# dpmerrell/PathMatFac.jl

Hardware: AMD Instinct MI355X
Metric: fit_iters_per_sec (higher is better)
Workload: dtype f32; 1 GPU; fit! epoch on synthetic 200000x50000 matrix (D stored as f32), K=64, Gaussian loss, group-reg X (32 groups) + featureset-ARD Y, adam; rows sharded over 1 GPU(s); full_model=False, M=200000, N=50000, K=64, rows_per_gpu=200000, optimizer=adam, parallelism=single GPU, rccl_ranks=0, collectives_issued=0, column_chunks=1

## Files before the change

include/pmf_hip.h:

```cpp
#ifndef PMF_HIP_H
#define PMF_HIP_H

#include <stdint.h>

#ifdef __cplusplus
extern "C" {
#endif

typedef struct pmf_ctx pmf_ctx;

#define PMF_NOISE_NORMAL 0
#define PMF_NOISE_BERNOULLI 1
#define PMF_NOISE_POISSON 2
#define PMF_NOISE_SQ_HINGE 3

#define PMF_OPT_ADAGRAD 0
#define PMF_OPT_ADAM 1

#define PMF_STORE_F32 0
#define PMF_STORE_BF16 1

#define PMF_TERM_MAX_EPOCHS 0
#define PMF_TERM_LOSS_INCREASE 1
#define PMF_TERM_ABS_TOL 2
// ... 134 lines not shown
int pmf_fit_lbfgs(pmf_ctx *ctx, const pmf_lbfgs_opts *opts, pmf_lbfgs_result *result);
int pmf_debug_lbfgs_direction(pmf_ctx *ctx, int n_pairs, const float *sX, const float *sY, const float *yX,
                              const float *yY, const float *gX, const float *gY, float *pX, float *pY);

int pmf_epoch_begin(pmf_ctx *ctx, const pmf_fit_opts *opts);
int pmf_epoch_step_local(pmf_ctx *ctx, const pmf_fit_opts *opts);
int pmf_epoch_step_shared(pmf_ctx *ctx, const pmf_fit_opts *opts);
int pmf_epoch_loss(pmf_ctx *ctx, double *local_loss, double *shared_terms);

#define PMF_COMM_ID_BYTES 128
#define PMF_COMM_NONE 0
#define PMF_COMM_RCCL 1
#define PMF_COMM_HOST 2
typedef int (*pmf_host_allreduce_fn)(void *user, void *host_buf, int64_t count, int dtype);
int pmf_comm_get_unique_id(void *id_out);
int pmf_comm_init(pmf_ctx *ctx, int rank, int nranks, const void *unique_id);
int pmf_comm_init_host(pmf_ctx *ctx, int rank, int nranks, pmf_host_allreduce_fn fn, void *user);
int pmf_comm_destroy(pmf_ctx *ctx);
int pmf_comm_set_chunks(pmf_ctx *ctx, int n_chunks);
int pmf_comm_allreduce(pmf_ctx *ctx, void *host_buf, int64_t count, int dtype, int op);
int pmf_comm_info(pmf_ctx *ctx, int *rank, int *nranks, int *transport, int *n_chunks, int *reserved_cus,
                  int64_t *n_collectives);

int pmf_debug_last_path(pmf_ctx *ctx, int *bmode, int *layer_path, int *slots, int *xreg, int64_t *plain_tiles);
int pmf_debug_plain_table(pmf_ctx *ctx, int32_t *out, int64_t cap, int64_t *n_rp, int64_t *n_ct);
int pmf_debug_last_kernel(pmf_ctx *ctx, int *kernel);

#define PMF_PASS_EXTENTS_MAX 16
int pmf_debug_pass_extents(pmf_ctx *ctx, int update_X, int update_Y, const int64_t *cap_override, int n_max,
                           const char **names, int64_t *need, int64_t *capacity, int *n);

int pmf_debug_live_bytes(int64_t *device_bytes, int64_t *pinned_bytes);

int pmf_grad_device_ptr(pmf_ctx *ctx, int which, void **ptr, int64_t *n_elements);
int pmf_get_grad(pmf_ctx *ctx, int which, int view, float *out);

int pmf_forward(pmf_ctx *ctx, float *Z_host);

#define PMF_IMPUTE_BATCH 1
#define PMF_IMPUTE_LINK 2
#define PMF_IMPUTE_KEEP_OBSERVED 4
int pmf_impute(pmf_ctx *ctx, int flags, int64_t row_start1, int64_t row_stop1, float *out_host, int64_t ld);
int pmf_impute_device(pmf_ctx *ctx, int flags, int64_t row_start1, int64_t row_stop1, float *out_device, int64_t ld);
int pmf_impute_entries(pmf_ctx *ctx, int flags, int64_t n, const int64_t *rows1, const int64_t *cols1, float *out_host);
int pmf_debug_impute_offset(int64_t row, int64_t col, int64_t ld, int64_t *offset);

typedef struct pmf_sim_opts {
// ... 73 lines not shown
```

pathmatfac.jl_amd/_lib.py:

```python
import ctypes as C
import os
from pathlib import Path

import numpy as np

_HERE = Path(__file__).resolve().parent
LIB_PATH = _HERE / "libpmf_hip.so"

NOISE = {"normal": 0, "bernoulli": 1, "poisson": 2, "bernoulli_sq_hinge": 3, "ordinal_sq_hinge3": 3}
HINGE_THRESHOLDS = {"bernoulli_sq_hinge": (0.0, np.inf, np.inf), "ordinal_sq_hinge3": (-np.inf, -0.5, 0.5)}
OPT = {"adagrad": 0, "adam": 1}
STORE = {"f32": 0, "bf16": 1}
TERM = {0: "max_epochs", 1: "loss_increase", 2: "abs_tol", 3: "rel_tol", 4: "nonfinite"}
IMPUTE_BATCH, IMPUTE_LINK, IMPUTE_KEEP_OBSERVED = 1, 2, 4
DEBATCH_LINK, DEBATCH_FILL_MISSING = 1, 2
PARAM = {"X": 0, "Y": 1, "logsigma": 2, "mu": 3, "logdelta": 4, "theta": 5}


class PMFError(RuntimeError):
    pass


class FitOpts(C.Structure):
    _fields_ = [("update_X", C.c_int32), ("update_Y", C.c_int32), ("update_col_layers", C.c_int32),
# ... 57 lines not shown
    L, Nv = S.shape
    flat = np.flatnonzero(S.ravel())
    rowptr = np.zeros(L + 1, np.int64)
    if Nv:
        np.cumsum(np.bincount(flat // Nv, minlength=L), out=rowptr[1:])
        col = (flat % Nv).astype(np.int32)
    else:
        col = np.zeros(0, np.int32)
    return rowptr, col, S.ravel()[flat].astype(np.float32)


EXPORTS = [
    "pmf_last_error", "pmf_version", "pmf_device_count", "pmf_create", "pmf_destroy", "pmf_set_stream", "pmf_synchronize",
    "pmf_set_data", "pmf_set_data_device", "pmf_set_factors", "pmf_set_X", "pmf_set_Y", "pmf_get_factors",
    "pmf_set_col_params", "pmf_get_col_params", "pmf_set_n_batch_views", "pmf_set_batch_view",
    "pmf_get_batch_view", "pmf_set_noise", "pmf_clear_xreg", "pmf_add_xreg_l2", "pmf_add_xreg_group",
    "pmf_clear_yreg", "pmf_add_yreg_l2", "pmf_add_yreg_group", "pmf_add_yreg_ard", "pmf_add_yreg_fsard",
    "pmf_set_layer_regs", "pmf_set_optimizer", "pmf_set_lr", "pmf_get_lr", "pmf_reset_optimizer_state",
    "pmf_fit", "pmf_epoch_begin", "pmf_epoch_step_local", "pmf_epoch_step_shared", "pmf_epoch_loss",
    "pmf_grad_device_ptr", "pmf_get_grad", "pmf_forward", "pmf_stats", "pmf_kernel_time", "pmf_synth_data",
    "pmf_set_precision", "pmf_get_precision",
    "pmf_comm_get_unique_id", "pmf_comm_init", "pmf_comm_init_host", "pmf_comm_destroy", "pmf_comm_set_chunks",
    "pmf_comm_info", "pmf_comm_allreduce", "pmf_get_opt_state", "pmf_fsard_update_A", "pmf_debug_last_path", "pmf_debug_last_kernel",
    "pmf_debug_pass_extents", "pmf_debug_live_bytes", "pmf_debug_plain_table",
    "pmf_add_xreg_network", "pmf_add_yreg_network", "pmf_get_reg_network_state", "pmf_add_xreg_l1", "pmf_add_yreg_l1",
    "pmf_impute", "pmf_impute_device", "pmf_impute_entries", "pmf_debug_impute_offset",
    "pmf_loss", "pmf_fit_lbfgs", "pmf_debug_lbfgs_direction",
    "pmf_stage_init_logsigma", "pmf_stage_reweight_col_losses", "pmf_get_noise_weights", "pmf_stage_minimal_group_weights",
    "pmf_stage_theta_delta_em",
    "pmf_gram", "pmf_stage_lambda_max", "pmf_stage_whiten", "pmf_stage_rotate_by_svd", "pmf_stage_reorder_by_importance",
    "pmf_debug_postprocess_times",
    "pmf_fsard_update_A_csr",
    "pmf_set_noise_thresholds", "pmf_get_noise_thresholds",
    "pmf_remove_batch_effect", "pmf_remove_batch_effect_device", "pmf_remove_batch_effect_entries",
    "pmf_simulate_data", "pmf_simulate_data_device", "pmf_simulate_data_resident",
]

COMM_ID_BYTES = 128
HOST_ALLREDUCE_FN = C.CFUNCTYPE(C.c_int, C.c_void_p, C.c_void_p, C.c_int64, C.c_int)


def comm_unique_id(lib_path=None):
    lib = load_library(lib_path)
    buf = C.create_string_buffer(COMM_ID_BYTES)
    if lib.pmf_comm_get_unique_id(buf) != 0:
        raise PMFError(lib.pmf_last_error().decode())
    return buf.raw
# ... 683 lines not shown

    def comm_destroy(self):
        self._chk(self.lib.pmf_comm_destroy(self._h))
        self._host_cb = None

    def comm_set_chunks(self, n):
        self._chk(self.lib.pmf_comm_set_chunks(self._h, int(n)))

    def comm_allreduce(self, arr, op="sum"):
        if arr.dtype not in (np.float32, np.float64) or not arr.flags.c_contiguous:
            raise PMFError("comm_allreduce needs a contiguous float32 / float64 array")
        self._chk(self.lib.pmf_comm_allreduce(self._h, arr.ctypes.data_as(C.c_void_p), C.c_int64(arr.size),
                                              1 if arr.dtype == np.float64 else 0, {"sum": 0, "max": 1}[op]))
        return arr

    def comm_info(self):
        r, n, t, ch, cu = C.c_int(0), C.c_int(0), C.c_int(0), C.c_int(0), C.c_int(0)
        nc = C.c_int64(0)
        self._chk(self.lib.pmf_comm_info(self._h, C.byref(r), C.byref(n), C.byref(t), C.byref(ch), C.byref(cu), C.byref(nc)))
        return dict(rank=r.value, nranks=n.value, transport=("none", "rccl", "host")[t.value], n_chunks=ch.value,
                    reserved_cus=cu.value, n_collectives=nc.value)

    def last_path(self):
        b, l, s, x = C.c_int(0), C.c_int(0), C.c_int(0), C.c_int(0)
        pt = C.c_int64(0)
        self._chk(self.lib.pmf_debug_last_path(self._h, C.byref(b), C.byref(l), C.byref(s), C.byref(x), C.byref(pt)))
        return dict(bmode=b.value, layer_path=l.value, slots=s.value, xreg=x.value, plain_tiles=pt.value)

    def plain_table(self):
        n_rp, n_ct = C.c_int64(0), C.c_int64(0)
        self._chk(self.lib.pmf_debug_plain_table(self._h, None, C.c_int64(0), C.byref(n_rp), C.byref(n_ct)))
        out = np.zeros((n_rp.value, n_ct.value + 1), np.int32)
        self._chk(self.lib.pmf_debug_plain_table(self._h, out.ctypes.data_as(C.c_void_p), C.c_int64(out.size), None, None))
        return out

    def last_kernel(self):
        k = C.c_int(0)
        self._chk(self.lib.pmf_debug_last_kernel(self._h, C.byref(k)))
        return k.value

    def pass_extents(self, update_X=False, update_Y=False, capacity_override=None):
        n_max = 16
        names, n = (C.c_char_p * n_max)(), C.c_int(0)
        need, cap = (C.c_int64 * n_max)(), (C.c_int64 * n_max)()
        ov = None
        if capacity_override is not None:
            plain = self.pass_extents(update_X, update_Y)
            unknown = set(capacity_override) - set(plain)
            if unknown:
                raise PMFError(f"pass_extents: unknown buffers {sorted(unknown)}")
# ... 23 lines not shown
```

pathmatfac.jl_amd/csrc/pmf_common.h:

```cpp
#ifndef PMF_COMMON_H
#define PMF_COMMON_H
#include <hip/hip_runtime.h>

#include <cstdint>
#include <type_traits>
#include <unordered_map>

#include "../../include/pmf_hip.h"

int pmf_fail(const char *fmt, ...);
#define HIPCHK(x)                                                                                    \
  do {                                                                                               \
    hipError_t e_ = (x);                                                                             \
    if (e_ != hipSuccess) return pmf_fail("%s failed: %s (%s:%d)", #x, hipGetErrorString(e_), __FILE__, __LINE__); \
  } while (0)
#define PMFCHK(x)          \
  do {                     \
    int r_ = (x);          \
    if (r_ < 0) return r_; \
  } while (0)

typedef std::unordered_map<const void *, size_t> PmfDynLds;
int pmf_ensure_dyn_lds(PmfDynLds *cache, const void *kern, size_t lds);

// ... 39 lines not shown
  const float2 *btab;
  const float2 *btd;
  const uint8_t *pm, *row_slot, *colview;
  int32_t nbs_shift;
  int32_t n_bv;
  double *loss_partial;
  int64_t M, N;
  int32_t n_cseg;
  int32_t want_gx, want_gy;
  unsigned long long *stamps;
  int32_t dbg;
  const ViewDesc *views;
  const char *Xsb, *Ysb;
  int32_t ct0;
  float *gx_part;
  const int32_t *piece_base;
  int64_t gx_slot_stride;
  const float *sb_scale_x, *sb_scale_y;
  const float *htab;
  const int32_t *ptab;
  int32_t ptab_stride;
  int32_t plain;
  int32_t *plain_count;
};

__device__ __forceinline__ int pmf_rowmap(int r, int h) { return (r & 3) + 8 * (r >> 2) + 4 * h; }
__device__ __forceinline__ bool pmf_finite(float y) { return fabsf(y) <= 3.402823466e38f; }

__host__ __device__ __forceinline__ int pmf_meta_kind(int meta) { return meta & 3; }
__host__ __device__ __forceinline__ int pmf_meta_view(int meta) { return (meta >> 2) - 1; }
__host__ __device__ __forceinline__ int64_t pmf_view_index(const ViewDesc &vd, int64_t j, int b) { return (j - vd.c0) * vd.nb + b; }
__host__ __device__ __forceinline__ int64_t pmf_btab_index(const ViewDesc &vd, int64_t j, int b) { return vd.tab_off + pmf_view_index(vd, j, b); }
__device__ __forceinline__ int pmf_row_batch(const int32_t *bor, int64_t M, int v, int64_t i) { return v >= 0 ? bor[(int64_t)v * M + i] : -1; }
__device__ __forceinline__ float2 pmf_batch_dt(const ViewDesc &vd, const float2 *btab, int64_t j, int b) {
  return b >= 0 ? btab[pmf_btab_index(vd, j, b)] : make_float2(1.f, 0.f);
}

#define PMF_HT 8
__device__ __forceinline__ void pmf_hinge_terms(float z, float y, const float *T, float &a, float &b) {
  const int c = (int)fminf(fmaxf(y + 0.5f, 0.f), 3.f);
  const float lo = T[c], hi = T[4 + c];
  a = fmaxf(0.f, 1.f - (z - lo));
  b = fmaxf(0.f, 1.f - (hi - z));
}
__device__ __forceinline__ float pmf_hinge_class(float z, const float4 t) { return (float)((t.x < z) + (t.y < z) + (t.z < z)); }

// ... 386 lines not shown
```

pathmatfac.jl_amd/csrc/pmf_ctx.h:

```cpp
#ifndef PMF_CTX_H
#define PMF_CTX_H
#include <hip/hip_runtime.h>

#include <algorithm>
#include <atomic>
#include <chrono>
#include <cmath>
#include <cstdarg>
#include <cstdio>
#include <cstdlib>
#include <cstring>
#include <memory>
#include <string>
#include <unordered_map>
#include <vector>

#include "pmf_common.h"

int memset_now(void *p, int v, size_t bytes);
inline std::atomic<int64_t> pmf_live_bytes[2];
template <typename T, bool PINNED = false>
struct DevBuf {
  T *p = nullptr;
  size_t n = 0;
// ... 123 lines not shown
  int64_t ptab_bm = 0, ptab_n_rp = 0, ptab_n_ct = 0;
  DevBuf<int32_t> plain_count;
  int64_t last_plain_n = -1;
  int store = PMF_STORE_F32;
  ParamBuf P[6];
  int n_bv = 0;
  std::vector<ViewDesc> views;
  std::vector<int64_t> val_off;
  std::vector<int64_t> bvb_off;
  DevBuf<int32_t> bor;
  DevBuf<float2> btab;
  bool views_dirty = true;
  DevBuf<ViewDesc> d_views;
  DevBuf<float2> LG;
  DevBuf<float> lgrad_part;
  DevBuf<float2> btd;
  bool btd_ok = false;
  int nbs = 16;
  DevBuf<uint8_t> colview;
  std::vector<std::vector<int32_t>> h_bor;
  PanelSlots pslots[3];
  int64_t views_serial = 0;
  int last_kernel = 0;
  int last_bmode = 0, last_layer_path = 0, last_xreg = 0;
  DevBuf<int32_t> d_val_view;
  DevBuf<int32_t> colmeta;
  DevBuf<float> colw;
  DevBuf<float4> colp;
  DevBuf<float4> thr;
  DevBuf<float> htab;
  std::vector<float> h_thr;
  bool mixed = false;
  bool prepared = false;
  DevBuf<float> ard_alpha, ard_beta;
  float ard_scale = 0.f;
  bool has_ard = false;
  bool ard_is_fsard = false;
  int opt_kind = PMF_OPT_ADAGRAD;
  float lr = 1.f, eps = 1e-8f, b1 = 0.9f, b2 = 0.999f;
  bool state_init = false;
  DevBuf<double> loss_partial;
  std::vector<uint8_t> h_kind;
  std::vector<int64_t> noise_s1, noise_e1;
  std::vector<WorkSplit> splits;
  int n_chunks_req = 0;
  DevBuf<float> gx_part;
  DevBuf<int32_t> gx_off, gx_idx;
// ... 152 lines not shown
```

pathmatfac.jl_amd/csrc/pmf_fused.hip.inc:

```

template <int KB, int NW, int RBW = 1>
struct FusedCfg {
  static constexpr int Kp = 32 * KB;
  static constexpr int KpS = Kp + 4;
  static constexpr int SLAB = 32 * Kp;
  static constexpr int YT = PMF_BN * KpS;
  static constexpr int XP = 32 * KpS;
  static constexpr int TT = (RBW - 1) * 1024;
  static constexpr int FIXED = NW * SLAB + NW * RBW * XP + NW * TT + 8 * PMF_BN + 4;
  static constexpr int LDS_BUDGET = 160 * 1024;
  static constexpr int NYB = (2 * YT + FIXED) * 4 + 8 * NW <= LDS_BUDGET ? 2 : 1;
  static constexpr size_t lds_bytes = (sizeof(float) * (NYB * YT + FIXED) + sizeof(double) * NW + 15) / 16 * 16;
  static constexpr size_t lds_batch_extra = PMF_BN * 16 * sizeof(float2) + PMF_PM_BYTES + NW * RBW * 16 * 32;
};

#ifndef PMF_NW4_WAVES
#define PMF_NW4_WAVES 1
#endif
#ifndef PMF_Y1BASE
#define PMF_Y1BASE 1
#endif
template <bool B> struct PmfFlag { static constexpr bool value = B; };
template <int KB, int NW, int RBW, int BMODE, bool MIXED, int GM, bool DB, bool XW = false, bool XR = false>
__global__ __launch_bounds__(64 * NW, (NW == 8 ? 2 : PMF_NW4_WAVES)) void pmf_fused_kernel(const FusedArgs a) {
// ... 94 lines not shown
    }
  }
  constexpr bool Y1BASE = PLAINB && PMF_Y1BASE != 0;
  unsigned g2_lane = (unsigned)(uintptr_t)(lds_cptr)(Ys + 4 * h * KpS + l31);
  if (Y1BASE) asm volatile("" : "+v"(g2_lane));
  auto ho_at = [](const void *base, unsigned &off) {
    if (PLAINB) asm volatile("" : "+v"(off));
    return reinterpret_cast<const char *>(base) + off;
  };
#ifdef PMF_STAMPS
  unsigned long long st_acc[16] = {0, 0, 0, 0, 0, 0, 0, 0, 0, 0, 0, 0, 0, 0, 0, 0};
  unsigned long long st_prev = __builtin_amdgcn_s_memtime();
  const unsigned long long st_t0 = st_prev, st_r0 = __builtin_amdgcn_s_memrealtime();
#endif
  const int wg = pmf_xcd_wg(blockIdx.x, gridDim.x);
  const int64_t w_begin = a.wg_begin[wg];
  const int64_t w_end = a.wg_begin[wg + 1];
  float *myslab = a.gy_slabs + (int64_t)wg * a.slab_stride;
  const int64_t seg_block = a.n_rp * a.tps;
  double lossacc = 0.0;
  int n_plain = 0;
  int seg_cur = -1, pidx = 0, t0_first = 0;
  int gx_slot = (GM == 2) ? 0 : a.piece_base[wg];
  for (int64_t widx = w_begin; widx < w_end;) {
    int cs = (int)(widx / seg_block);
    if (cs > a.n_cseg - 1) cs = a.n_cseg - 1;
    const int tps_cs = cs == a.n_cseg - 1 ? a.n_ct - (a.n_cseg - 1) * a.tps : a.tps;
    const int64_t rem = widx - (int64_t)cs * seg_block;
    const int64_t rp = rem / tps_cs;
    const int ti0 = (int)(rem - rp * tps_cs);
    const int ntiles = (int)(tps_cs - ti0 < w_end - widx ? tps_cs - ti0 : w_end - widx);
    widx += ntiles;
    if (cs != seg_cur) { seg_cur = cs; pidx = 0; t0_first = ti0; } else { ++pidx; }
    bool slab_first = true;
    int pl_b = ntiles, pl_e = ntiles;
    int32_t pl_c0 = 0, pl_c1 = 0;
    if (PLAINB && a.plain) {
      const int64_t c_abs = (int64_t)a.ct0 + (int64_t)cs * a.tps + ti0;
      const bool rag = (c_abs + ntiles) * PMF_BN > N;
      pl_b = pidx == 0 ? ntiles : (pidx == 1 ? (t0_first - ti0 < 0 ? 0 : (t0_first - ti0 < ntiles ? t0_first - ti0 : ntiles)) : 0);
      pl_e = rag ? ntiles - 2 : ntiles;
      if (pl_b < pl_e) {
        const int32_t *pt = a.ptab + rp * a.ptab_stride;
        pl_c0 = pt[c_abs + pl_b];
        pl_c1 = pt[c_abs + (rag ? ntiles - 1 : ntiles)];
      } else {
        pl_b = pl_e = ntiles;
      }
    }
    const int64_t col_begin = ((int64_t)a.ct0 + (int64_t)cs * a.tps + ti0) * BN;
    int64_t row0[RBW], irow_c[RBW];
    bool row_ok[RBW];
#pragma unroll
    for (int rb = 0; rb < RBW; ++rb) {
      row0[rb] = rp * BM + (int64_t)(w * RBW + rb) * 32;
      const int64_t irow = row0[rb] + l31;
      row_ok[rb] = irow < M;
      irow_c[rb] = row_ok[rb] ? irow : (M - 1);
    }

    constexpr int XV = (32 * Kp / 4) / 64;
    float4 xv0[RBW][XV];
#pragma unroll
    for (int rb = 0; rb < RBW; ++rb) {
#pragma unroll
      for (int q = 0; q < XV; ++q) {
        const int e4 = lane + 64 * q;
        const int il = (e4 * 4) / Kp;
        const int64_t ir = row0[rb] + il < M ? row0[rb] + il : M - 1;
        xv0[rb][q] = *reinterpret_cast<const float4 *>(a.X + ir * Kp + (e4 * 4) % Kp);
      }
    }
    f32x16 gx[RBW][KB];
#pragma unroll
    for (int rb = 0; rb < RBW; ++rb)
#pragma unroll
      for (int kb = 0; kb < KB; ++kb)
#pragma unroll
        for (int r = 0; r < 16; ++r) gx[rb][kb][r] = 0.f;
    float4 xf[XR ? KS / 4 : 1];
    float xg[XR ? 8 * NW : 1];

    auto stage_load_y = [&](int64_t jt, int q, float4 (&yv)[YV], float (&sgv)[YV], bool plain = false) {
      const float *yb = a.Y + jt * Kp;
      const float4 *cb = a.colp + jt;
      const int64_t rem = N - jt;
      if (HOIST && !(PLAINB && !plain && rem < BN)) {
        const bool rag = HOZ == 2 && rem < BN;
        yv[q] = *reinterpret_cast<const float4 *>(ho_at(yb, rag ? ho_y[HOZ - 1][q] : ho_y[0][q]));
        sgv[q] = *reinterpret_cast<const float *>(ho_at(cb, rag ? ho_s[HOZ - 1][q] : ho_s[0][q]));
        return;
      }
      const int ncol = rem > BN ? BN : (int)rem;
      int e4 = tid + NT * q;
// ... 150 lines not shown
        const int64_t rem = N - jt_red;
        const int nel = (rem > BN ? BN : (int)rem) * Kp;
        float *sb = myslab + jt_red * Kp;
#pragma unroll
        for (int q = 0; q < RV4; ++q) {
          float4 v = racc[q];
          const float sgj = Csg[(cbuf ^ 1) * BN + eo[q] / Kp];
          v.x *= sgj; v.y *= sgj; v.z *= sgj; v.w *= sgj;
          if (!slab_first) { v.x += gold[q].x; v.y += gold[q].y; v.z += gold[q].z; v.w += gold[q].w; }
          if (in[q] && eo[q] < nel) pmf_store_stream(reinterpret_cast<float4 *>(sb + eo[q]), v);
        }
      }
    };

    bool rows_in[RBW];
    int rb_u[RBW];
    uint32_t tflag[RBW];
#pragma unroll
    for (int rb = 0; rb < RBW; ++rb) {
      const int rb_raw = __builtin_amdgcn_readfirstlane((int)(row0[rb] >> 5));
      rows_in[rb] = rb_raw < a.nRB;
      rb_u[rb] = rows_in[rb] ? rb_raw : (int)a.nRB - 1;
      tflag[rb] = a.tflags[(col_begin >> 5) * a.nRB + rb_u[rb]];
#pragma unroll
      for (int q = 0; q < DCH; ++q) dcur[rb].load(a.D, (col_begin >> 5) * a.nRB + rb_u[rb], lane, q);
    }
    {
      float4 yv[YV], cv;
      float sgv[YV];
      stage_load(col_begin, yv, sgv, cv);
#pragma unroll
      for (int rb = 0; rb < RBW; ++rb)
#pragma unroll
        for (int q = 0; q < XV; ++q) {
          const int e4 = lane + 64 * q;
          const int il = (e4 * 4) / Kp, kf = (e4 * 4) % Kp;
          *reinterpret_cast<float4 *>(Xw[rb] + il * KpS + kf) = row0[rb] + il < M ? xv0[rb][q] : make_float4(0.f, 0.f, 0.f, 0.f);
        }
      stage_store(0, 0, col_begin, yv, sgv, cv);
      if (bt_lds) {
#pragma unroll
        for (int q = 0; q < NBT; ++q) {
          const int e = bt_e(q);
          bt_store(e, pmf_bt_entry(a, a.pm + rp * a.n_bv * 16, col_begin, e, pmf_bt_view(a, col_begin, e)), bt_mu(col_begin, e));
        }
        if (tid < a.n_bv * 16) Pm[tid] = a.pm[rp * a.n_bv * 16 + tid];
        if (h == 0)
#pragma unroll
          for (int rb = 0; rb < RBW; ++rb)
            for (int v = 0; v < a.n_bv; ++v) Bw0[rb * 512 + v * 32 + l31] = a.row_slot[(int64_t)v * M + irow_c[rb]];
      }
    }
    __syncthreads();
    if (XR) {
      const float4 *xr0 = reinterpret_cast<const float4 *>(Xw[0] + l31 * KpS + h * (Kp / 2));
#pragma unroll
      for (int q = 0; q < KS / 4; ++q) xf[XR ? q : 0] = xr0[q];
#pragma unroll
      for (int q = 0; q < 8 * NW; ++q) {
        const int p = q >> 3, u = (q >> 1) & 3, hi = q & 1;
        xg[XR ? q : 0] = *(lds_cptr)(uintptr_t)(xw_xa[u] + 4 * (p * Cfg::XP + 16 * hi * KpS));
      }
    }

    f32x16 acc[RBW];
    forward_reduce(acc, 0, 0, false, 0);

    int t_plain = ntiles, t_pend = ntiles;
    if (PLAINB && a.plain) {
      const bool run = pl_b < pl_e && pl_c0 == pl_c1;
      t_plain = __builtin_amdgcn_readfirstlane(run ? pl_b : ntiles);
      t_pend = __builtin_amdgcn_readfirstlane(run ? pl_e : ntiles);
      n_plain += t_pend - t_plain;
    }
    auto tile_loop = [&](auto plain_flag, const int t_begin, const int t_end) __attribute__((always_inline)) {
    constexpr bool PLAIN = decltype(plain_flag)::value;
    for (int t = t_begin; t < t_end; ++t) {
      const int par = t & 1;
      const int cur = NYB == 2 ? par : 0, nxt = NYB == 2 ? (par ^ 1) : 0;
      const int64_t j0 = col_begin + (int64_t)t * BN;
      const float *Yc = Ys + cur * Cfg::YT;
      const bool have_next = (t + 1 < ntiles);
      const int cb0 = par * BN + 4 * h;
      float4 ynext[YV], cnext;
      float2 btn[NBT];
      float btm[NBT];
      int btv[NBT];
      float sgnext[YV];
      PMF_STAMP(0);
      const float xw_sg = XW ? Csg[par * BN + xw_j] : 0.f;

      float lsum = 0.f;
      const int tkind = MIXED ? __builtin_amdgcn_readfirstlane(Ck[par]) : 0;
      const int tview = bt_lds ? __builtin_amdgcn_readfirstlane(Ck[2 + par]) : -1;
      float lnorm = 0.f;
      auto epi_reg = [&](int rb, int r, float dl, float th, float wj, int kmode, bool fast) __attribute__((always_inline)) {
        if (dbg & 4) return;
        float z = acc[rb][r];
        if (BATCH) z = fmaf(z, dl, th);
        float y = dcur[rb].get(r);
        if (kmode == PMF_NOISE_NORMAL) {
// ... 28 lines not shown
              dv[u] = Btd[bsr * 32 + cl];
              tv[u] = Btt[bsr * 32 + cl];
            } else {
              tv[u] = Cmu[par * BN + cl];
              if (v >= 0) {
                const int64_t vc0 = a.views[v].c0, vto = a.views[v].tab_off;
                const int vnb = a.views[v].nb;
                const int b = a.bor[(int64_t)v * M + irow_c[rb]];
                if (b >= 0) {
                  const float2 dt = a.btab[vto + (j0 + cl - vc0) * vnb + b];
                  dv[u] = dt.x;
                  tv[u] += dt.y;
                }
              }
            }
          }
          dl4 = make_float4(dv[0], dv[1], dv[2], dv[3]);
          th4 = make_float4(tv[0], tv[1], tv[2], tv[3]);
        }
      };
      const float4 *cw4 = reinterpret_cast<const float4 *>(Cw + cb0);
      auto f4get = [](const float4 &v, int u) { return u == 0 ? v.x : (u == 1 ? v.y : (u == 2 ? v.z : v.w)); };

      const int64_t jn = have_next ? j0 + BN : j0;
      constexpr int NOTH = YV + 1 + RV4 + (BATCH ? NBT : 0);
      constexpr int DPR = DCH + (PLAIN ? 0 : 1);
      constexpr int NVM = NOTH + DPR * RBW;
      bool tile_fast[RBW];
#pragma unroll
      for (int rb = 0; rb < RBW; ++rb) tile_fast[rb] = PLAIN || (rows_in[rb] && tflag[rb] != 0);
      auto vmem_op = [&](int i) {
        if (i == 0 && bt_lds) {
#pragma unroll
          for (int q = 0; q < NBT; ++q) btv[q] = pmf_bt_view(a, jn, bt_e(q));
        }
        if (i < YV) stage_load_y(jn, i, ynext, sgnext, PLAIN);
        else if (i == YV) stage_load_c(jn, cnext, PLAIN);
        else if (i < YV + 1 + RV4) { if (want_gy) slab_prefetch_one(j0, i - YV - 1, PLAIN); }
        else if (i < NOTH) {
          const int q = i - YV - 1 - RV4;
          if (bt_lds) { btn[q] = pmf_bt_entry(a, Pm, jn, bt_e(q), btv[q]); btm[q] = bt_mu(jn, bt_e(q)); }
        }
        else if (i < NVM) {
          const int rb = (i - NOTH) / DPR, q = (i - NOTH) % DPR;
          if (q < DCH) {
            if (FULL || !(dbg & 2)) dcur[rb].load(a.D, (jn >> 5) * a.nRB + rb_u[rb], lane, q);
          } else {
            tflag[rb] = a.tflags[(jn >> 5) * a.nRB + rb_u[rb]];
          }
        }
      };
      typedef float f32x2 __attribute__((ext_vector_type(2)));
#pragma unroll
      for (int rb = 0; rb < RBW; ++rb) {
        if (!BATCH && tile_fast[rb] && (!MIXED || tkind == 0)) {
          f32x2 ls2 = {0.f, 0.f};
          if (!(dbg & 4)) {
#pragma unroll
            for (int c4 = 0; c4 < 4; ++c4) {
              const float4 w4 = cw4[2 * c4];
#pragma unroll
              for (int p2 = 0; p2 < 2; ++p2) {
                const int r = 4 * c4 + 2 * p2;
                const f32x2 zz = {acc[rb][r], acc[rb][r + 1]}, yy = {dcur[rb].get(r), dcur[rb].get(r + 1)};
                const f32x2 ww = p2 == 0 ? f32x2{w4.x, w4.y} : f32x2{w4.z, w4.w};
                f32x2 dd;
                asm("v_pk_add_f32 %0, %1, %2 neg_lo:[0,1] neg_hi:[0,1]" : "=v"(dd) : "v"(zz), "v"(yy));
                const f32x2 gg = ww * dd;
                ls2 = gg * dd + ls2;
                acc[rb][r] = gg.x; acc[rb][r + 1] = gg.y;
              }
// ... 138 lines not shown
            if (!XR) xa[(q + hi) % XW_RING] = *(lds_cptr)(uintptr_t)((TIGHT ? xt_xa[u] : xw_xa[u]) + 4 * (p * Cfg::XP + 16 * hi * KpS));
            xb[(q + hi) % XW_RING] = Gp[p * 1024 + (TIGHT ? xt_g[u] : xw_g[u]) + 512 * hi];
          }
        };
#pragma unroll
        for (int q = 0; q < XW_AHEAD; q += 2) xw_read(q);
        f32x4 gy0 = {0.f, 0.f, 0.f, 0.f}, gy1 = {0.f, 0.f, 0.f, 0.f};
        __builtin_amdgcn_sched_barrier(0);
#pragma unroll
        for (int q = 0; q < 8 * NW; q += 2) {
          if (q + XW_AHEAD < 8 * NW) xw_read(q + XW_AHEAD);
          gy0 = __builtin_amdgcn_mfma_f32_16x16x4f32(XR ? xg[XR ? q : 0] : xa[q % XW_RING], xb[q % XW_RING], gy0, 0, 0, 0);
          gy1 = __builtin_amdgcn_mfma_f32_16x16x4f32(XR ? xg[XR ? q + 1 : 0] : xa[(q + 1) % XW_RING], xb[(q + 1) % XW_RING], gy1, 0, 0, 0);
          __builtin_amdgcn_sched_barrier(0);
        }
        dcur[0].touch();
        const int64_t rem = N - j0;
        const int nel = (rem > BN ? BN : (int)rem) * Kp;
        float4 v = make_float4((gy0[0] + gy1[0]) * xw_sg, (gy0[1] + gy1[1]) * xw_sg, (gy0[2] + gy1[2]) * xw_sg, (gy0[3] + gy1[3]) * xw_sg);
        if (!slab_first) { v.x += gold[0].x; v.y += gold[0].y; v.z += gold[0].z; v.w += gold[0].w; }
        if (PLAIN) pmf_store_stream(reinterpret_cast<float4 *>(const_cast<char *>(ho_at(myslab + j0 * Kp, ho_g[0][0]))), v);
        else if (xw_e < nel) pmf_store_stream(reinterpret_cast<float4 *>(myslab + j0 * Kp + xw_e), v);
        PMF_STAMP(4);
        forward_reduce(acc, nxt, par ^ 1, false, 0);
        PMF_STAMP(8);
        if (bt_lds) __syncthreads();
        PMF_STAMP(9);
      } else {
        if (FULL || have_next) forward_reduce(acc, nxt, par ^ 1, want_gy && !(dbg & 1), j0);
        else if (want_gy && !(dbg & 1)) { f32x16 dummy[RBW]; forward_reduce(dummy, nxt, par ^ 1, true, j0); }
        PMF_STAMP(8);
        if ((GM != 1 || bt_lds) && !(dbg & 16)) __syncthreads();
        PMF_STAMP(9);
      }
    }
    };
    if constexpr (PLAINB) {
      tile_loop(PmfFlag<false>{}, 0, t_plain);
      tile_loop(PmfFlag<PLAINB>{}, t_plain, t_pend);
      if (t_pend < ntiles) {
#pragma unroll
        for (int rb = 0; rb < RBW; ++rb) tflag[rb] = 1;
        tile_loop(PmfFlag<false>{}, t_pend, ntiles);
      }
    } else {
      tile_loop(PmfFlag<false>{}, 0, ntiles);
    }
    if (XW && !bt_lds) __syncthreads();

    PMF_STAMP(10);
    if (want_gx) {
      float *gp = a.gx_part + (int64_t)gx_slot * a.gx_slot_stride + (int64_t)(w * RBW) * 32 * Kp + l31;
#pragma unroll
      for (int rb = 0; rb < RBW; ++rb)
#pragma unroll
        for (int kb = 0; kb < KB; ++kb)
#pragma unroll
          for (int r = 0; r < 16; ++r) gp[(rb * 32 + pmf_rowmap(r, h)) * Kp + 32 * kb] = gx[rb][kb][r];
    }
    ++gx_slot;
    PMF_STAMP(11);
  }
#pragma unroll
  for (int off = 32; off > 0; off >>= 1) lossacc += __shfl_xor(lossacc, off, 64);
  if (lane == 0) red[w] = lossacc;
  __syncthreads();
  if (tid == 0) {
    double s = 0.0;
    for (int q = 0; q < NW; ++q) s += red[q];
    a.loss_partial[wg] = s;
    if (PLAINB && a.plain_count) a.plain_count[wg] = n_plain;
  }
#ifdef PMF_STAMPS
  st_acc[14] = __builtin_amdgcn_s_memtime() - st_t0;
  st_acc[15] = __builtin_amdgcn_s_memrealtime() - st_r0;
  if (a.stamps && (threadIdx.x & 63) == 0) {
    for (int q = 0; q < 16; ++q) a.stamps[((int64_t)blockIdx.x * NW + (threadIdx.x >> 6)) * 16 + q] = st_acc[q];
  }
#endif
}
```

pathmatfac.jl_amd/csrc/pmf_pass.hip:

```cpp
#include "pmf_ctx.h"

__global__ void k_tile_flags(const void *__restrict__ D, int64_t ntiles, uint32_t *__restrict__ flags, int bf16) {
  const int64_t t = blockIdx.x;
  if (t >= ntiles) return;
  bool ok;
  if (bf16) {
    const uint2 v = reinterpret_cast<const uint2 *>(reinterpret_cast<const uint16_t *>(D) + t * 1024)[threadIdx.x];
    ok = (v.x & 0x7f80u) != 0x7f80u && (v.x & 0x7f800000u) != 0x7f800000u && (v.y & 0x7f80u) != 0x7f80u && (v.y & 0x7f800000u) != 0x7f800000u;
  } else {
    const float4 v = reinterpret_cast<const float4 *>(reinterpret_cast<const float *>(D) + t * 1024)[threadIdx.x];
    ok = fabsf(v.x) <= 3.402823466e38f && fabsf(v.y) <= 3.402823466e38f && fabsf(v.z) <= 3.402823466e38f && fabsf(v.w) <= 3.402823466e38f;
  }
  const int all_ok = __syncthreads_and(ok ? 1 : 0);
  if (threadIdx.x == 0) flags[t] = all_ok ? 1u : 0u;
}

static int ensure_tile_flags(pmf_ctx *c) {
  if (c->tflags_valid) return 0;
  const int64_t ntiles = c->nRB * (c->D_Npad / 32);
  PMFCHK(c->tflags.ensure((size_t)ntiles, false));
  if (ntiles > 0x7fffffff) return pmf_fail("too many tiles");
  k_tile_flags<<<(unsigned)ntiles, 256, 0, c->stream>>>(c->D, ntiles, c->tflags, c->store == PMF_STORE_BF16);
  HIPCHK(hipGetLastError());
  c->tflags_valid = true;
// ... 538 lines not shown
  for (int q = 0; q < s; ++q) loss_off += c->splits[(size_t)q].grid;
  FusedArgs a;
  memset(&a, 0, sizeof(a));
  a.tflags = c->tflags;
  a.wg_begin = ws.wg_begin;
  a.D = c->D; a.X = c->P[0].p; a.Y = c->P[1].p; a.gX = c->P[0].g; a.gY = c->P[1].g;
  a.colp = c->colp; a.htab = c->htab; a.bor = c->bor; a.btab = c->btab; a.loss_partial = c->loss_partial + loss_off;
  a.btd = g.bmode == 1 ? c->btd : nullptr; a.n_bv = c->n_bv;
  if (g.bmode == 1) {
    a.pm = g.ps->pm; a.row_slot = g.ps->row_slot; a.colview = c->colview;
    a.nbs_shift = 0;
    while ((1 << a.nbs_shift) < c->nbs) ++a.nbs_shift;
  }
  c->last_bmode = g.bmode;
  a.nRB = c->nRB; a.gy_slabs = c->gy_slabs; a.slab_stride = slab_stride; a.n_rp = n_rp;
  a.M = c->M; a.N = c->N; a.n_tiles = n_rp * n_ct; a.tps = (int)tiles_per_seg; a.n_ct = (int)n_ct; a.n_cseg = (int)n_cseg;
  a.want_gx = want_gx; a.want_gy = want_gy;
  a.ct0 = (int32_t)g.ct0[s];
  const bool has_plain = pass_has_plain_loop(c, g, want_gx, want_gy);
  if (has_plain) {
    const char *pe = getenv("PMF_PLAIN");
    a.ptab = c->ptab; a.ptab_stride = (int32_t)(g.n_ct_all + 1); a.plain = !(pe && atoi(pe) == 0);
    a.plain_count = c->plain_count + loss_off;
  }
  a.gx_part = c->gx_part; a.piece_base = ws.d_piece_base_abs; a.gx_slot_stride = (int64_t)f.BM() * c->Kp;
  {
    const char *dbg = getenv("PMF_DEBUG_FLAGS");
    a.dbg = dbg ? atoi(dbg) : 0;
  }
#ifdef PMF_STAMPS
  {
    static DevBuf<unsigned long long> d_stamps;
    PMFCHK(d_stamps.ensure((size_t)16 * 8 * 1024, false));
    HIPCHK(hipMemsetAsync(d_stamps, 0, sizeof(unsigned long long) * 16 * 8 * 1024, c->stream));
    a.stamps = d_stamps;
    g_stamps = d_stamps;
  }
#endif
  a.views = c->d_views;
  const bool batch = c->n_bv > 0;
  if (f.img != IMG_NONE) {
    if (s == 0) PMFCHK(sb_split_x(c, f));
    PMFCHK(sb_split_y(c, f, g.ct0[s], n_ct, s));
    a.Xsb = c->xsb; a.Ysb = c->ysb;
    if (f.img == IMG_SB8) { a.sb_scale_x = c->sb8_scale; a.sb_scale_y = c->sb8_scale + 1 + s; }
  }
  if (c->ev_used == c->ev_pool.size()) {
    if (c->ev_pool.size() >= 4096) {
      HIPCHK(hipStreamSynchronize(c->stream));
      harvest_events(c);
    } else {
      hipEvent_t e0, e1;
      HIPCHK(hipEventCreate(&e0));
      HIPCHK(hipEventCreate(&e1));
      c->ev_pool.emplace_back(e0, e1);
    }
  }
  auto &ev = c->ev_pool[c->ev_used++];
  HIPCHK(hipEventRecord(ev.first, c->stream));
  c->last_kernel = f.kernel;
  pmf_last_xreg = 0;
  const int rc = f.launch[c->store == PMF_STORE_BF16](&c->dyn_lds, c->stream, a, grid, batch, c->mixed);
  c->last_xreg = pmf_last_xreg;
  c->last_plain_n = has_plain && pmf_last_xreg ? loss_off + grid : -1;
  if (f.kernel != 0) c->sb_launches += 1;
  PMFCHK(rc);
  HIPCHK(hipEventRecord(ev.second, c->stream));
  if (want_gy && !(a.dbg & 8)) {
    k_gy_reduce<<<dim3((unsigned)n_ct, (unsigned)(32 * c->Kp / 256)), 64, 0, c->stream>>>(c->gy_slabs, slab_stride, ws.c_off, ws.c_idx,
                                                                                      c->Kp, c->N, c->P[1].g, (int)g.ct0[s],
                                                                                      f.img == IMG_SB8 ? c->colp : nullptr);
    HIPCHK(hipGetLastError());
  }
  if (want_gx && s == g.S - 1) {
    const int64_t panel = (int64_t)f.BM() * c->Kp;
    k_gx_reduce<<<dim3((unsigned)g.n_rp, (unsigned)((panel / 4 + 255) / 256)), 256, 0, c->stream>>>(
        c->gx_part, panel, c->gx_off, c->gx_idx, panel, (int64_t)c->Kp * c->M, c->P[0].g);
    HIPCHK(hipGetLastError());
  }
  return 0;
}

int launch_fused(pmf_ctx *c, bool want_gx, bool want_gy) {
  const FusedGeom g = fused_geometry(c, want_gx, want_gy, c->n_chunks_req > 0);
  PMFCHK(prepare_fused_pass(c, g, want_gx, want_gy));
  PMFCHK(guard_fused_pass(c, g, want_gx, want_gy));
  for (int s = 0; s < g.S; ++s) PMFCHK(launch_fused_chunk(c, g, s, want_gx, want_gy));
  return 0;
}

thread_local int pmf_last_xreg = 0;
extern "C" int pmf_debug_last_kernel(pmf_ctx *c, int *kernel) {
  if (!c) return pmf_fail("null context");
  if (kernel) *kernel = c->last_kernel;
  return 0;
}

extern "C" int pmf_debug_last_path(pmf_ctx *c, int *bmode, int *layer_path, int *slots, int *xreg, int64_t *plain_tiles) {
  if (!c) return pmf_fail("null context");
  if (plain_tiles) {
    *plain_tiles = 0;
    if (c->last_plain_n > 0) {
      PMFCHK(ctx_bind(c));
      std::vector<int32_t> h((size_t)c->last_plain_n);
      HIPCHK(hipMemcpyAsync(h.data(), c->plain_count, h.size() * sizeof(int32_t), hipMemcpyDeviceToHost, c->stream));
      HIPCHK(hipStreamSynchronize(c->stream));
      for (int32_t v : h) *plain_tiles += v;
    }
  }
  if (xreg) *xreg = c->last_xreg;
  if (bmode) *bmode = c->last_bmode;
  if (layer_path) *layer_path = c->last_layer_path;
  if (slots) *slots = c->nbs;
  return 0;
}

extern "C" int pmf_debug_plain_table(pmf_ctx *c, int32_t *out, int64_t cap, int64_t *n_rp, int64_t *n_ct) {
  PMFCHK(ctx_bind(c));
  if (!c->D) return pmf_fail("data not set");
  PMFCHK(ensure_tile_flags(c));
  const int64_t nct = (c->N + PMF_BN - 1) / PMF_BN;
  PMFCHK(ensure_plain_table(c, 256, nct));
  if (n_rp) *n_rp = c->ptab_n_rp;
  if (n_ct) *n_ct = nct;
  if (out) {
    const int64_t n = c->ptab_n_rp * (nct + 1);
    if (cap < n) return pmf_fail("pmf_debug_plain_table: room for %lld entries, %lld needed", (long long)cap, (long long)n);
    HIPCHK(hipMemcpyAsync(out, c->ptab, (size_t)n * sizeof(int32_t), hipMemcpyDeviceToHost, c->stream));
    HIPCHK(hipStreamSynchronize(c->stream));
  }
  return 0;
}

extern "C" int pmf_debug_pass_extents(pmf_ctx *c, int update_X, int update_Y, const int64_t *cap_override, int n_max,
                                      const char **names, int64_t *need, int64_t *capacity, int *n_out) {
  PMFCHK(ctx_bind(c));
  PMFCHK(check_ready(c));
  if (!c->prepared) PMFCHK(prepare(c));
  const bool want_gx = update_X != 0, want_gy = update_Y != 0;
  const FusedGeom g = fused_geometry(c, want_gx, want_gy, c->n_chunks_req > 0);
  PMFCHK(prepare_fused_pass(c, g, want_gx, want_gy));
  PassExtent e[PMF_PASS_EXTENTS];
  const int n = fused_pass_extents(c, g, want_gx, want_gy, e);
  if (n_max < n) return pmf_fail("pmf_debug_pass_extents: room for %d entries, %d needed", n_max, n);
  for (int i = 0; i < n; ++i) {
    if (cap_override && cap_override[i] >= 0) e[i].cap = cap_override[i];
    if (names) names[i] = e[i].name;
    if (need) need[i] = e[i].need;
    if (capacity) capacity[i] = e[i].cap;
  }
  if (n_out) *n_out = n;
// ... 3 lines not shown
```

Measured before the change: 33.31 iters/s.

## Prefetch next piece's X rows and D tile across work-piece seams in fused kernel

In the plain-B fused kernel, each wave now finds the next work piece while finishing the current one. During the last tile it prefetches the next piece's D tile and X rows into registers, and it skips the end-of-piece sync and re-staging so the next piece starts warm. This targets the per-piece startup latency of reloading X and D and redoing stage loads at seams. In exchange it adds register pressure from the held xv_seam and d_seam copies and makes the tile-parity bookkeeping more complex. A PMF_SEAM env var can turn it off, and debug hooks for the work split are added.

```diff
diff --git a/include/pmf_hip.h b/include/pmf_hip.h
--- a/include/pmf_hip.h
+++ b/include/pmf_hip.h
@@ -180,7 +180,8 @@
 int pmf_comm_info(pmf_ctx *ctx, int *rank, int *nranks, int *transport, int *n_chunks, int *reserved_cus,
                   int64_t *n_collectives);
 
-int pmf_debug_last_path(pmf_ctx *ctx, int *bmode, int *layer_path, int *slots, int *xreg, int64_t *plain_tiles);
+int pmf_debug_last_path(pmf_ctx *ctx, int *bmode, int *layer_path, int *slots, int *xreg, int64_t *plain_tiles, int *seam);
+int pmf_debug_work_split(pmf_ctx *ctx, int update_X, int update_Y, int chunk, int64_t *wg_begin, int64_t cap, int64_t *geom);
 int pmf_debug_plain_table(pmf_ctx *ctx, int32_t *out, int64_t cap, int64_t *n_rp, int64_t *n_ct);
 int pmf_debug_last_kernel(pmf_ctx *ctx, int *kernel);
 
diff --git a/pathmatfac.jl_amd/_lib.py b/pathmatfac.jl_amd/_lib.py
--- a/pathmatfac.jl_amd/_lib.py
+++ b/pathmatfac.jl_amd/_lib.py
@@ -103,7 +103,7 @@
     "pmf_set_precision", "pmf_get_precision",
     "pmf_comm_get_unique_id", "pmf_comm_init", "pmf_comm_init_host", "pmf_comm_destroy", "pmf_comm_set_chunks",
     "pmf_comm_info", "pmf_comm_allreduce", "pmf_get_opt_state", "pmf_fsard_update_A", "pmf_debug_last_path", "pmf_debug_last_kernel",
-    "pmf_debug_pass_extents", "pmf_debug_live_bytes", "pmf_debug_plain_table",
+    "pmf_debug_pass_extents", "pmf_debug_live_bytes", "pmf_debug_plain_table", "pmf_debug_work_split",
     "pmf_add_xreg_network", "pmf_add_yreg_network", "pmf_get_reg_network_state", "pmf_add_xreg_l1", "pmf_add_yreg_l1",
     "pmf_impute", "pmf_impute_device", "pmf_impute_entries", "pmf_debug_impute_offset",
     "pmf_loss", "pmf_fit_lbfgs", "pmf_debug_lbfgs_direction",
@@ -833,10 +833,19 @@
                     reserved_cus=cu.value, n_collectives=nc.value)
 
     def last_path(self):
-        b, l, s, x = C.c_int(0), C.c_int(0), C.c_int(0), C.c_int(0)
+        b, l, s, x, sm = C.c_int(0), C.c_int(0), C.c_int(0), C.c_int(0), C.c_int(0)
         pt = C.c_int64(0)
-        self._chk(self.lib.pmf_debug_last_path(self._h, C.byref(b), C.byref(l), C.byref(s), C.byref(x), C.byref(pt)))
-        return dict(bmode=b.value, layer_path=l.value, slots=s.value, xreg=x.value, plain_tiles=pt.value)
+        self._chk(self.lib.pmf_debug_last_path(self._h, C.byref(b), C.byref(l), C.byref(s), C.byref(x), C.byref(pt), C.byref(sm)))
+        return dict(bmode=b.value, layer_path=l.value, slots=s.value, xreg=x.value, plain_tiles=pt.value, seam=sm.value)
+
+    def work_split(self, update_X=False, update_Y=False, chunk=0):
+        geom = (C.c_int64 * 8)()
+        self._chk(self.lib.pmf_debug_work_split(self._h, int(update_X), int(update_Y), int(chunk), None, C.c_int64(0), geom))
+        wb = np.zeros(int(geom[0]) + 1, np.int64)
+        self._chk(self.lib.pmf_debug_work_split(self._h, int(update_X), int(update_Y), int(chunk), wb.ctypes.data_as(C.c_void_p),
+                                                C.c_int64(wb.size), geom))
+        keys = ("grid", "n_rp", "n_ct", "tps", "n_cseg", "ct0", "chunks", "n_cu")
+        return dict(wg_begin=wb, **{k: int(v) for k, v in zip(keys, geom)})
 
     def plain_table(self):
         n_rp, n_ct = C.c_int64(0), C.c_int64(0)
diff --git a/pathmatfac.jl_amd/csrc/pmf_common.h b/pathmatfac.jl_amd/csrc/pmf_common.h
--- a/pathmatfac.jl_amd/csrc/pmf_common.h
+++ b/pathmatfac.jl_amd/csrc/pmf_common.h
@@ -85,6 +85,7 @@
   int32_t ptab_stride;
   int32_t plain;
   int32_t *plain_count;
+  int32_t seam;
 };
 
 __device__ __forceinline__ int pmf_rowmap(int r, int h) { return (r & 3) + 8 * (r >> 2) + 4 * h; }
diff --git a/pathmatfac.jl_amd/csrc/pmf_ctx.h b/pathmatfac.jl_amd/csrc/pmf_ctx.h
--- a/pathmatfac.jl_amd/csrc/pmf_ctx.h
+++ b/pathmatfac.jl_amd/csrc/pmf_ctx.h
@@ -169,7 +169,7 @@
   PanelSlots pslots[3];
   int64_t views_serial = 0;
   int last_kernel = 0;
-  int last_bmode = 0, last_layer_path = 0, last_xreg = 0;
+  int last_bmode = 0, last_layer_path = 0, last_xreg = 0, last_seam = 0;
   DevBuf<int32_t> d_val_view;
   DevBuf<int32_t> colmeta;
   DevBuf<float> colw;
diff --git a/pathmatfac.jl_amd/csrc/pmf_fused.hip.inc b/pathmatfac.jl_amd/csrc/pmf_fused.hip.inc
--- a/pathmatfac.jl_amd/csrc/pmf_fused.hip.inc
+++ b/pathmatfac.jl_amd/csrc/pmf_fused.hip.inc
@@ -140,16 +140,39 @@
   int n_plain = 0;
   int seg_cur = -1, pidx = 0, t0_first = 0;
   int gx_slot = (GM == 2) ? 0 : a.piece_base[wg];
-  for (int64_t widx = w_begin; widx < w_end;) {
-    int cs = (int)(widx / seg_block);
+  auto piece_at = [&](int64_t wi, int &cs, int64_t &rp, int &ti0, int &ntiles) {
+    cs = (int)(wi / seg_block);
     if (cs > a.n_cseg - 1) cs = a.n_cseg - 1;
     const int tps_cs = cs == a.n_cseg - 1 ? a.n_ct - (a.n_cseg - 1) * a.tps : a.tps;
-    const int64_t rem = widx - (int64_t)cs * seg_block;
-    const int64_t rp = rem / tps_cs;
-    const int ti0 = (int)(rem - rp * tps_cs);
-    const int ntiles = (int)(tps_cs - ti0 < w_end - widx ? tps_cs - ti0 : w_end - widx);
+    const int64_t rem = wi - (int64_t)cs * seg_block;
+    rp = rem / tps_cs;
+    ti0 = (int)(rem - rp * tps_cs);
+    ntiles = (int)(tps_cs - ti0 < w_end - wi ? tps_cs - ti0 : w_end - wi);
+  };
+  static_assert(!PLAINB || RBW == 1, "seams: one row block per wave");
+  const bool seam_on = PLAINB && a.seam != 0;
+  bool warm = false;
+  int poff = 0;
+  constexpr int XV = (32 * Kp / 4) / 64;
+  float4 xv_seam[XV];
+  PmfDTile<DB> d_seam;
+  for (int64_t widx = w_begin; widx < w_end;) {
+    int cs, ti0, ntiles;
+    int64_t rp;
+    piece_at(widx, cs, rp, ti0, ntiles);
     widx += ntiles;
     if (cs != seg_cur) { seg_cur = cs; pidx = 0; t0_first = ti0; } else { ++pidx; }
+    const bool more = seam_on && widx < w_end;
+    int64_t jn_last = ((int64_t)a.ct0 + (int64_t)cs * a.tps + ti0 + ntiles - 1) * PMF_BN;
+    int rb_nx = __builtin_amdgcn_readfirstlane((int)rp * NW + w);
+    if (PLAINB && more) {
+      int nx_cs, nx_ti0, nx_nt;
+      int64_t nx_rp;
+      piece_at(widx, nx_cs, nx_rp, nx_ti0, nx_nt);
+      jn_last = ((int64_t)a.ct0 + (int64_t)nx_cs * a.tps + nx_ti0) * PMF_BN;
+      rb_nx = __builtin_amdgcn_readfirstlane((int)nx_rp * NW + w);
+    }
+    const int t_brk = more ? ntiles : 0x7fffffff;
     bool slab_first = true;
     int pl_b = ntiles, pl_e = ntiles;
     int32_t pl_c0 = 0, pl_c1 = 0;
@@ -157,7 +180,7 @@
       const int64_t c_abs = (int64_t)a.ct0 + (int64_t)cs * a.tps + ti0;
       const bool rag = (c_abs + ntiles) * PMF_BN > N;
       pl_b = pidx == 0 ? ntiles : (pidx == 1 ? (t0_first - ti0 < 0 ? 0 : (t0_first - ti0 < ntiles ? t0_first - ti0 : ntiles)) : 0);
-      pl_e = rag ? ntiles - 2 : ntiles;
+      pl_e = rag ? ntiles - 2 : (PLAINB && more && jn_last + PMF_BN > N ? ntiles - 1 : ntiles);
       if (pl_b < pl_e) {
         const int32_t *pt = a.ptab + rp * a.ptab_stride;
         pl_c0 = pt[c_abs + pl_b];
@@ -177,17 +200,22 @@
       irow_c[rb] = row_ok[rb] ? irow : (M - 1);
     }
 
-    constexpr int XV = (32 * Kp / 4) / 64;
     float4 xv0[RBW][XV];
-#pragma unroll
-    for (int rb = 0; rb < RBW; ++rb) {
+    auto x_issue = [&](float4 (&xv)[XV], int64_t r0, int ln) {
 #pragma unroll
       for (int q = 0; q < XV; ++q) {
-        const int e4 = lane + 64 * q;
+        const int e4 = ln + 64 * q;
         const int il = (e4 * 4) / Kp;
-        const int64_t ir = row0[rb] + il < M ? row0[rb] + il : M - 1;
-        xv0[rb][q] = *reinterpret_cast<const float4 *>(a.X + ir * Kp + (e4 * 4) % Kp);
-      }
+        const int64_t ir = r0 + il < M ? r0 + il : M - 1;
+        xv[q] = *reinterpret_cast<const float4 *>(a.X + ir * Kp + (e4 * 4) % Kp);
+      }
+    };
+    if (PLAINB && warm) {
+#pragma unroll
+      for (int q = 0; q < XV; ++q) xv0[0][q] = xv_seam[q];
+    } else {
+#pragma unroll
+      for (int rb = 0; rb < RBW; ++rb) x_issue(xv0[rb], row0[rb], lane);
     }
     f32x16 gx[RBW][KB];
 #pragma unroll
@@ -384,13 +412,14 @@
       rows_in[rb] = rb_raw < a.nRB;
       rb_u[rb] = rows_in[rb] ? rb_raw : (int)a.nRB - 1;
       tflag[rb] = a.tflags[(col_begin >> 5) * a.nRB + rb_u[rb]];
+      if (PLAINB && warm) {
+        dcur[rb] = d_seam;
+        continue;
+      }
 #pragma unroll
       for (int q = 0; q < DCH; ++q) dcur[rb].load(a.D, (col_begin >> 5) * a.nRB + rb_u[rb], lane, q);
     }
-    {
-      float4 yv[YV], cv;
-      float sgv[YV];
-      stage_load(col_begin, yv, sgv, cv);
+    if (PLAINB && warm) {
 #pragma unroll
       for (int rb = 0; rb < RBW; ++rb)
 #pragma unroll
@@ -399,7 +428,21 @@
           const int il = (e4 * 4) / Kp, kf = (e4 * 4) % Kp;
           *reinterpret_cast<float4 *>(Xw[rb] + il * KpS + kf) = row0[rb] + il < M ? xv0[rb][q] : make_float4(0.f, 0.f, 0.f, 0.f);
         }
-      stage_store(0, 0, col_begin, yv, sgv, cv);
+    } else {
+      float4 yv[YV], cv;
+      float sgv[YV];
+      stage_load(col_begin, yv, sgv, cv);
+#pragma unroll
+      for (int rb = 0; rb < RBW; ++rb)
+#pragma unroll
+        for (int q = 0; q < XV; ++q) {
+          const int e4 = lane + 64 * q;
+          const int il = (e4 * 4) / Kp, kf = (e4 * 4) % Kp;
+          *reinterpret_cast<float4 *>(Xw[rb] + il * KpS + kf) = row0[rb] + il < M ? xv0[rb][q] : make_float4(0.f, 0.f, 0.f, 0.f);
+        }
+      int zb = 0;
+      if (PLAINB) asm volatile("" : "+s"(zb));
+      stage_store(zb, zb, col_begin, yv, sgv, cv);
       if (bt_lds) {
 #pragma unroll
         for (int q = 0; q < NBT; ++q) {
@@ -426,7 +469,8 @@
     }
 
     f32x16 acc[RBW];
-    forward_reduce(acc, 0, 0, false, 0);
+    forward_reduce(acc, PLAINB ? poff : 0, PLAINB ? poff : 0, false, 0);
+    PMF_STAMP(12);
 
     int t_plain = ntiles, t_pend = ntiles;
     if (PLAINB && a.plain) {
@@ -435,10 +479,10 @@
       t_pend = __builtin_amdgcn_readfirstlane(run ? pl_e : ntiles);
       n_plain += t_pend - t_plain;
     }
-    auto tile_loop = [&](auto plain_flag, const int t_begin, const int t_end) __attribute__((always_inline)) {
+    auto tile_loop = [&](auto plain_flag, const int t_begin, const int t_end) __attribute__((always_inline)) -> bool {
     constexpr bool PLAIN = decltype(plain_flag)::value;
     for (int t = t_begin; t < t_end; ++t) {
-      const int par = t & 1;
+      const int par = (PLAINB ? t + poff : t) & 1;
       const int cur = NYB == 2 ? par : 0, nxt = NYB == 2 ? (par ^ 1) : 0;
       const int64_t j0 = col_begin + (int64_t)t * BN;
       const float *Yc = Ys + cur * Cfg::YT;
@@ -513,7 +557,10 @@
       const float4 *cw4 = reinterpret_cast<const float4 *>(Cw + cb0);
       auto f4get = [](const float4 &v, int u) { return u == 0 ? v.x : (u == 1 ? v.y : (u == 2 ? v.z : v.w)); };
 
-      const int64_t jn = have_next ? j0 + BN : j0;
+      const int64_t jn = have_next ? j0 + BN : (PLAINB ? jn_last : j0);
+      int rb_n[RBW];
+#pragma unroll
+      for (int rb = 0; rb < RBW; ++rb) rb_n[rb] = PLAINB && !have_next ? (rb_nx < a.nRB ? rb_nx : (int)a.nRB - 1) : rb_u[rb];
       constexpr int NOTH = YV + 1 + RV4 + (BATCH ? NBT : 0);
       constexpr int DPR = DCH + (PLAIN ? 0 : 1);
       constexpr int NVM = NOTH + DPR * RBW;
@@ -535,9 +582,9 @@
         else if (i < NVM) {
           const int rb = (i - NOTH) / DPR, q = (i - NOTH) % DPR;
           if (q < DCH) {
-            if (FULL || !(dbg & 2)) dcur[rb].load(a.D, (jn >> 5) * a.nRB + rb_u[rb], lane, q);
+            if (FULL || !(dbg & 2)) dcur[rb].load(a.D, (jn >> 5) * a.nRB + rb_n[rb], lane, q);
           } else {
-            tflag[rb] = a.tflags[(jn >> 5) * a.nRB + rb_u[rb]];
+            tflag[rb] = a.tflags[(jn >> 5) * a.nRB + rb_n[rb]];
           }
         }
       };
@@ -722,6 +769,7 @@
         if (PLAIN) pmf_store_stream(reinterpret_cast<float4 *>(const_cast<char *>(ho_at(myslab + j0 * Kp, ho_g[0][0]))), v);
         else if (xw_e < nel) pmf_store_stream(reinterpret_cast<float4 *>(myslab + j0 * Kp + xw_e), v);
         PMF_STAMP(4);
+        if (PLAINB && t + 1 == t_brk) return true;
         forward_reduce(acc, nxt, par ^ 1, false, 0);
         PMF_STAMP(8);
         if (bt_lds) __syncthreads();
@@ -734,11 +782,10 @@
         PMF_STAMP(9);
       }
     }
+    return false;
     };
     if constexpr (PLAINB) {
-      tile_loop(PmfFlag<false>{}, 0, t_plain);
-      tile_loop(PmfFlag<PLAINB>{}, t_plain, t_pend);
-      if (t_pend < ntiles) {
+      if (!tile_loop(PmfFlag<false>{}, 0, t_plain) && !tile_loop(PmfFlag<PLAINB>{}, t_plain, t_pend) && t_pend < ntiles) {
 #pragma unroll
         for (int rb = 0; rb < RBW; ++rb) tflag[rb] = 1;
         tile_loop(PmfFlag<false>{}, t_pend, ntiles);
@@ -746,19 +793,37 @@
     } else {
       tile_loop(PmfFlag<false>{}, 0, ntiles);
     }
-    if (XW && !bt_lds) __syncthreads();
+    if (XW && !bt_lds && !(PLAINB && more)) __syncthreads();
+    if (PLAINB) {
+      d_seam = dcur[0];
+      if (more) {
+        int lo = lane;
+        asm volatile("" : "+v"(lo));
+        x_issue(xv_seam, (int64_t)rb_nx * 32, lo);
+      } else {
+#pragma unroll
+        for (int q = 0; q < XV; ++q) xv_seam[q] = make_float4(0.f, 0.f, 0.f, 0.f);
+      }
+    }
 
     PMF_STAMP(10);
     if (want_gx) {
-      float *gp = a.gx_part + (int64_t)gx_slot * a.gx_slot_stride + (int64_t)(w * RBW) * 32 * Kp + l31;
+      int lo = lane;
+      if (PLAINB) asm volatile("" : "+v"(lo));
+      const int fl31 = PLAINB ? lo & 31 : l31, fh = PLAINB ? lo >> 5 : h, fw = PLAINB ? __builtin_amdgcn_readfirstlane(w) : w;
+      float *gp = a.gx_part + (int64_t)gx_slot * a.gx_slot_stride + (int64_t)(fw * RBW) * 32 * Kp + fl31;
 #pragma unroll
       for (int rb = 0; rb < RBW; ++rb)
 #pragma unroll
         for (int kb = 0; kb < KB; ++kb)
 #pragma unroll
-          for (int r = 0; r < 16; ++r) gp[(rb * 32 + pmf_rowmap(r, h)) * Kp + 32 * kb] = gx[rb][kb][r];
+          for (int r = 0; r < 16; ++r) gp[(rb * 32 + pmf_rowmap(r, fh)) * Kp + 32 * kb] = gx[rb][kb][r];
     }
     ++gx_slot;
+    if (PLAINB) {
+      warm = more;
+      poff = more ? (poff + ntiles) & 1 : 0;
+    }
     PMF_STAMP(11);
   }
 #pragma unroll
diff --git a/pathmatfac.jl_amd/csrc/pmf_pass.hip b/pathmatfac.jl_amd/csrc/pmf_pass.hip
--- a/pathmatfac.jl_amd/csrc/pmf_pass.hip
+++ b/pathmatfac.jl_amd/csrc/pmf_pass.hip
@@ -584,6 +584,8 @@
     const char *pe = getenv("PMF_PLAIN");
     a.ptab = c->ptab; a.ptab_stride = (int32_t)(g.n_ct_all + 1); a.plain = !(pe && atoi(pe) == 0);
     a.plain_count = c->plain_count + loss_off;
+    const char *se = getenv("PMF_SEAM");
+    a.seam = !(se && atoi(se) == 0);
   }
   a.gx_part = c->gx_part; a.piece_base = ws.d_piece_base_abs; a.gx_slot_stride = (int64_t)f.BM() * c->Kp;
   {
@@ -625,6 +627,7 @@
   const int rc = f.launch[c->store == PMF_STORE_BF16](&c->dyn_lds, c->stream, a, grid, batch, c->mixed);
   c->last_xreg = pmf_last_xreg;
   c->last_plain_n = has_plain && pmf_last_xreg ? loss_off + grid : -1;
+  c->last_seam = has_plain && pmf_last_xreg && a.seam ? 1 : 0;
   if (f.kernel != 0) c->sb_launches += 1;
   PMFCHK(rc);
   HIPCHK(hipEventRecord(ev.second, c->stream));
@@ -658,8 +661,9 @@
   return 0;
 }
 
-extern "C" int pmf_debug_last_path(pmf_ctx *c, int *bmode, int *layer_path, int *slots, int *xreg, int64_t *plain_tiles) {
+extern "C" int pmf_debug_last_path(pmf_ctx *c, int *bmode, int *layer_path, int *slots, int *xreg, int64_t *plain_tiles, int *seam) {
   if (!c) return pmf_fail("null context");
+  if (seam) *seam = c->last_seam;
   if (plain_tiles) {
     *plain_tiles = 0;
     if (c->last_plain_n > 0) {
@@ -689,6 +693,29 @@
     const int64_t n = c->ptab_n_rp * (nct + 1);
     if (cap < n) return pmf_fail("pmf_debug_plain_table: room for %lld entries, %lld needed", (long long)cap, (long long)n);
     HIPCHK(hipMemcpyAsync(out, c->ptab, (size_t)n * sizeof(int32_t), hipMemcpyDeviceToHost, c->stream));
+    HIPCHK(hipStreamSynchronize(c->stream));
+  }
+  return 0;
+}
+
+extern "C" int pmf_debug_work_split(pmf_ctx *c, int update_X, int update_Y, int chunk, int64_t *wg_begin, int64_t cap, int64_t *geom) {
+  PMFCHK(ctx_bind(c));
+  PMFCHK(check_ready(c));
+  if (!c->prepared) PMFCHK(prepare(c));
+  const bool want_gx = update_X != 0, want_gy = update_Y != 0;
+  const FusedGeom g = fused_geometry(c, want_gx, want_gy, c->n_chunks_req > 0);
+  PMFCHK(prepare_fused_pass(c, g, want_gx, want_gy));
+  if (chunk < 0 || chunk >= g.S) return pmf_fail("pmf_debug_work_split: chunk %d of %d", chunk, g.S);
+  const WorkSplit &ws = c->splits[(size_t)chunk];
+  int grid; int64_t tps, n_cseg;
+  chunk_segments(c, g, chunk, grid, tps, n_cseg);
+  if (geom) {
+    const int64_t v[8] = {ws.grid, g.n_rp, g.nct[chunk], tps, n_cseg, g.ct0[chunk], g.S, c->n_cu};
+    memcpy(geom, v, sizeof(v));
+  }
+  if (wg_begin) {
+    if (cap < ws.grid + 1) return pmf_fail("pmf_debug_work_split: room for %lld entries, %lld needed", (long long)cap, (long long)ws.grid + 1);
+    HIPCHK(hipMemcpyAsync(wg_begin, ws.wg_begin, sizeof(int64_t) * ((size_t)ws.grid + 1), hipMemcpyDeviceToHost, c->stream));
     HIPCHK(hipStreamSynchronize(c->stream));
   }
   return 0;
```

After: 33.45 iters/s (median of 6 runs). About the same (+0.4%).
